# ChanganVR/RelationalGraphLearning

Hardware: AMD Instinct MI355X
Metric: agent-graph forward evals/sec (N=20, 2-layer GCN, depth-2 tree) (higher is better)
Workload: dtype f32 (24-bit operands throughout; 13 312 of the 14 224 products of the children kernel's 32 x 32, 32 x 100 and 100 x 100 head matrices, its embedding / graph weight products (w_r's second layer, Wa, W1, W_last) and the state predictor's weight products as six bf16 MFMA terms over three round-to-neare

## Files before the change

include/rgl_hip.h:

```cpp
#ifndef RGL_HIP_H
#define RGL_HIP_H

#include <stddef.h>

#ifdef __cplusplus
extern "C" {
#endif

#define RGL_ABI_VERSION 8

#define RGL_MAX_MLP_LAYERS 6
#define RGL_MAX_GCN_LAYERS 8
#define RGL_MAX_NODES 128
#define RGL_MAX_XDIM 64
#define RGL_MAX_WIDTH 256
#define RGL_MAX_ACTIONS 256

#define RGL_OK 0
#define RGL_ERR_BAD_SHAPE (-1)
#define RGL_ERR_BAD_MODE (-2)
#define RGL_ERR_NULL (-3)
#define RGL_ERR_WORKSPACE (-4)
#define RGL_CONTRACT_F32 0
#define RGL_CONTRACT_F16 1
// ... 123 lines not shown
    int planning_width;
    int do_action_clip;
    int sparse_search;
    int contraction_dtype;
    double time_step;
    double gamma_bar;
    const double* actions;
    const int* action_groups;
    const double* root_robot_f64;
    const double* root_humans_f64;
    const float* children_image;
    const float* predictor_image;
    double action_speed_bound;
} MprlPlanner;

size_t mprl_children_image_bytes(const MprlPlanner* planner);
int mprl_pack_children_image_f32(const MprlPlanner* planner, float* image, size_t image_bytes, rgl_stream_t stream);
size_t mprl_predictor_image_bytes(const MprlPlanner* planner);
int mprl_pack_predictor_image_f32(const MprlPlanner* planner, float* image, size_t image_bytes, rgl_stream_t stream);

int mprl_expand_f32(const MprlPlanner* planner, const float* robot, const float* humans, int P, int H,
                    int parents_are_joint_states,
                    float* humans_next, float* child_robot, float* reward, float* child_value,
                    float* value1, void* workspace, size_t workspace_bytes, rgl_stream_t stream);

size_t mprl_value_children_workspace_bytes(const MprlPlanner* planner, int P, int H);
int mprl_value_children_f32(const MprlPlanner* planner, const float* child_robot, const float* humans_next,
                            int P, int H, float* child_value, void* workspace, size_t workspace_bytes,
                            rgl_stream_t stream);

// ... 86 lines not shown
```

relationalgraphlearning_amd/_native.py:

```python
import ctypes as C
import os

_HERE = os.path.dirname(os.path.abspath(__file__))
LIB_PATH = os.environ.get("RGL_HIP_LIBRARY") or os.path.join(_HERE, "lib", "librgl_hip.so")

MAX_MLP_LAYERS = 6
MAX_GCN_LAYERS = 8
MAX_NODES = 128
MAX_XDIM = 64
MAX_WIDTH = 256
MAX_ACTIONS = 256
ABI_VERSION = 8
MSE_WORKSPACE_BYTES = 2048

SIMILARITY = {"embedded_gaussian": 0, "gaussian": 1, "cosine": 2, "cosine_softmax": 3, "concatenation": 4,
              "squared": 5, "equal_attention": 6, "diagonal": 7}
KINEMATICS = {"holonomic": 0, "unicycle": 1}
CONTRACTION_DTYPES = {"f32": 0, "f16": 1, "bf16x6": 3}

ERRORS = {-1: "RGL_ERR_BAD_SHAPE", -2: "RGL_ERR_BAD_MODE", -3: "RGL_ERR_NULL", -4: "RGL_ERR_WORKSPACE",
          -5: "RGL_ERR_LDS"}

c_float_p = C.POINTER(C.c_float)
c_int_p = C.POINTER(C.c_int)
# ... 9 lines not shown
    _fields_ = [("src", C.c_void_p), ("dst", C.c_void_p), ("rows", C.c_int), ("cols", C.c_int)]


class RglGatherJob(C.Structure):
    _fields_ = [("src", C.c_void_p), ("dst", C.c_void_p), ("row_floats", C.c_int), ("src_rows", C.c_int)]


class RglRowsPlan(C.Structure):
    _fields_ = [("kind", C.c_int), ("coop", C.c_int), ("waves_per_wg", C.c_int), ("n_waves", C.c_int), ("n_tiles", C.c_int),
                ("n_wgs", C.c_int), ("direct", C.c_int), ("reserved", C.c_int), ("lds_bytes", C.c_size_t)]


class RglGraphTilesPlan(C.Structure):
    _fields_ = [("covered", C.c_int), ("node_tiles", C.c_int), ("feature_tiles", C.c_int), ("layers", C.c_int), ("family", C.c_int),
                ("norm", C.c_int), ("grid", C.c_int), ("resident", C.c_int), ("lds_bytes", C.c_size_t)]


class RglGraph(C.Structure):
    _fields_ = [("w_r", RglMlp), ("w_h", RglMlp), ("x_dim", C.c_int), ("num_layer", C.c_int),
                ("similarity", C.c_int), ("layerwise_graph", C.c_int), ("skip_connection", C.c_int),
                ("reserved", C.c_int), ("w_a", C.c_void_p), ("w_a_mlp", RglMlp),
                ("Ws", C.c_void_p * MAX_GCN_LAYERS)]


class GcnPlanner(C.Structure):
    _fields_ = [("graph", RglGraph), ("value_head", RglMlp), ("kinematics", C.c_int), ("num_actions", C.c_int),
                ("time_step", C.c_double), ("gamma", C.c_double), ("actions", C.c_void_p),
                ("root_robot_f64", C.c_void_p), ("root_humans_f64", C.c_void_p), ("contraction_dtype", C.c_int), ("reserved", C.c_int)]


# ... 39 lines not shown


SIGNATURES = {
    "rgl_graph_forward_workspace_bytes": (C.c_size_t, [C.POINTER(RglGraph), C.POINTER(RglMlp), C.POINTER(RglMlp), C.c_int,
                                                       C.c_int, C.c_int]),
    "rgl_graph_forward_f32": (C.c_int, [C.POINTER(RglGraph), C.POINTER(RglMlp), C.POINTER(RglMlp), C.c_void_p,
                                        C.c_void_p, C.c_int, C.c_int, C.c_int, C.c_void_p, C.c_void_p, C.c_void_p,
                                        C.c_void_p, C.c_void_p, C.c_size_t, C.c_void_p]),
    "rgl_graph_param_count": (C.c_int, [C.POINTER(RglGraph), C.POINTER(RglMlp), C.POINTER(RglMlp)]),
    "rgl_graph_backward_workspace_bytes": (C.c_size_t, [C.POINTER(RglGraph), C.POINTER(RglMlp), C.POINTER(RglMlp), C.c_int]),
    "rgl_graph_backward_f32": (C.c_int, [C.POINTER(RglGraph), C.POINTER(RglMlp), C.POINTER(RglMlp), C.c_void_p, C.c_void_p,
                                         C.c_int, C.c_int, C.c_int, C.c_void_p, C.c_void_p, C.c_void_p, C.c_void_p,
                                         C.c_void_p, C.c_size_t, C.c_void_p]),
    "rgl_plan_mlp_rows": (C.c_int, [C.POINTER(RglMlp), C.c_int, C.c_int, C.POINTER(RglRowsPlan)]),
    "rgl_plan_graph_tiles": (C.c_int, [C.POINTER(RglGraph), C.c_int, C.c_int, C.c_int, C.c_int, C.POINTER(RglGraphTilesPlan)]),
    "rgl_transpose_f32": (C.c_int, [C.c_void_p, C.c_void_p, C.c_int, C.c_int, C.c_void_p]),
    "rgl_transpose_many_f32": (C.c_int, [C.c_void_p, C.c_int, C.c_void_p]),
    "rgl_gather_rows_f32": (C.c_int, [C.c_void_p, C.c_int, C.c_void_p, C.c_int, C.c_void_p]),
    "rgl_mse_step_f32": (C.c_int, [C.c_void_p, C.c_void_p, C.c_void_p, C.c_void_p, C.c_float, C.c_int, C.c_void_p, C.c_void_p,
                                   C.c_void_p, C.c_void_p]),
    "gcn_rotate_f32": (C.c_int, [C.c_void_p, C.c_void_p, C.c_int, C.c_int, C.c_void_p]),
    "gcn_prepare_f32": (C.c_int, [C.POINTER(GcnPlanner), C.c_void_p, C.c_void_p, C.c_int, C.c_int, C.c_void_p, C.c_void_p,
                                  C.c_void_p, C.c_void_p]),
    "gcn_predict_workspace_bytes": (C.c_size_t, [C.c_int, C.c_int, C.c_int]),
    "gcn_predict_f32": (C.c_int, [C.POINTER(GcnPlanner), C.c_void_p, C.c_void_p, C.c_int, C.c_int, C.c_void_p,
                                  C.c_size_t, C.c_void_p, C.c_void_p, C.c_void_p, C.c_void_p]),
    "mprl_expand_f32": (C.c_int, [C.POINTER(MprlPlanner), C.c_void_p, C.c_void_p, C.c_int, C.c_int, C.c_int,
                                  C.c_void_p, C.c_void_p, C.c_void_p, C.c_void_p, C.c_void_p, C.c_void_p, C.c_size_t,
                                  C.c_void_p]),
    "mprl_value_children_workspace_bytes": (C.c_size_t, [C.POINTER(MprlPlanner), C.c_int, C.c_int]),
# ... 17 lines not shown
    "mprl_tree_level_view": (C.c_int, [C.POINTER(MprlPlanner), C.c_int, C.c_int, C.c_int, C.POINTER(MprlLevelView)]),
    "crowd_step_f64": (C.c_int, [C.POINTER(CrowdSimConfig), C.c_void_p, C.c_void_p, C.c_void_p, C.c_void_p, C.c_void_p,
                                 C.c_void_p, C.c_void_p, C.c_void_p, C.c_int, C.c_int, C.c_int, C.c_void_p, C.c_void_p,
                                 C.c_void_p, C.c_void_p]),
    "crowd_observe_f32": (C.c_int, [C.c_void_p, C.c_void_p, C.c_int, C.c_int, C.c_void_p, C.c_void_p, C.c_void_p]),
    "crowd_orca_humans_f64": (C.c_int, [C.POINTER(CrowdOrcaParams), C.c_void_p, C.c_void_p, C.c_void_p, C.c_void_p,
                                        C.c_void_p, C.c_int, C.c_int, C.c_int, C.c_void_p, C.c_void_p]),
    "crowd_orca_robot_f64": (C.c_int, [C.POINTER(CrowdOrcaParams), C.c_void_p, C.c_void_p, C.c_void_p, C.c_int, C.c_int,
                                       C.c_void_p, C.c_void_p]),
    "crowd_generate_scenes_f64": (C.c_int, [C.POINTER(CrowdSceneConfig), C.c_void_p, C.c_int, C.c_int, C.c_void_p, C.c_void_p,
                                            C.c_void_p, C.c_void_p, C.c_void_p, C.c_void_p, C.c_void_p]),
    "rgl_abi_version": (C.c_int, []),
    "rgl_build_target": (C.c_char_p, []),
}

_lib = None


class NativeLibraryError(RuntimeError):
    pass


def lib():
    global _lib
    if _lib is None:
        if not os.path.exists(LIB_PATH):
            raise NativeLibraryError(
                "librgl_hip.so is not built (%s). Run `python -c 'import __graft_entry__ as g; g.build()'` or "
                "`make -C relationalgraphlearning_amd/csrc`. There is no CPU fallback." % LIB_PATH)
        handle = C.CDLL(LIB_PATH)
        for name, (res, args) in SIGNATURES.items():
            try:
                fn = getattr(handle, name)
            except AttributeError as e:
                raise NativeLibraryError("librgl_hip.so lacks symbol %s" % name) from e
            fn.restype = res
            fn.argtypes = args
        if handle.rgl_abi_version() != ABI_VERSION:
            raise NativeLibraryError("librgl_hip.so ABI %d != expected %d" % (handle.rgl_abi_version(), ABI_VERSION))
        _lib = handle
    return _lib


def poison_workspaces():
    return os.environ.get("RGL_DEBUG_POISON_WORKSPACES", "0") == "1"


def check(rc, what):
    if rc == 0:
# ... 5 lines not shown
```

relationalgraphlearning_amd/csrc/rgl_common.h:

```cpp
#pragma once
#include <hip/hip_runtime.h>

#include <cstdlib>

#include "rgl_hip.h"

#define RGL_HIP_TRY(expr)                          \
    do {                                           \
        hipError_t e__ = (expr);                   \
        if (e__ != hipSuccess) return (int)e__;    \
    } while (0)

#define RGL_LAUNCH_CHECK()                         \
    do {                                           \
        hipError_t e__ = hipGetLastError();        \
        if (e__ != hipSuccess) return (int)e__;    \
    } while (0)

namespace rgl {

constexpr int kLdsBytesPerCu = 160 * 1024;

inline int validate_mlp(const RglMlp& m, int want_in, int want_out) {
    if (m.n_layers < 1 || m.n_layers > RGL_MAX_MLP_LAYERS) return RGL_ERR_BAD_SHAPE;
// ... 57 lines not shown
                         hipStream_t stream, int mode = 0);
size_t fused_children_workspace_bytes(int P, int A, int H);
const float* fused_workspace_image(const void* workspace, size_t workspace_bytes);
int launch_value_children(const MprlPlanner* pl, const float* child_robot, const float* humans_next, int P, int H,
                          float* child_value, void* workspace, size_t workspace_bytes, hipStream_t stream,
                          int image_ready = 0, const void* tail = nullptr, size_t tail_bytes = 0,
                          int* tail_done = nullptr, const void* prologue = nullptr, size_t prologue_bytes = 0);
size_t value_children_workspace_bytes(const MprlPlanner* pl, int P, int H);
int launch_predict_humans(const MprlPlanner* pl, const float* robot, const float* humans, int crowds_per, int P, int H,
                          float* humans_next, void* workspace, size_t workspace_bytes, hipStream_t stream,
                          const void* children = nullptr, size_t children_bytes = 0, int* children_done = nullptr,
                          const float* sp_image = nullptr);
int level_prologue_args(const MprlPlanner* pl, const float* robot, const float* humans, int crowds_per, int P, int H,
                        float* humans_next, const float* sp_image, const void* children, size_t children_bytes, void* out,
                        size_t out_bytes);
bool fused_prologue_fits(const MprlPlanner* pl, int P, int H, size_t workspace_bytes, int scene_floats);
size_t scene_image_bytes(const MprlPlanner* pl);
int pack_scene_image(const MprlPlanner* pl, float* image, hipStream_t stream);
size_t scene_image_bytes_for(const RglGraph& g, const RglMlp* motion_head);
int pack_scene_image_for(const RglGraph& g, const RglMlp* motion_head, float* image, hipStream_t stream);

int launch_scene_children(const MprlPlanner* pl, const float* child_robot, const float* humans_next, int P, int H,
                          float* child_value, void* workspace, size_t workspace_bytes, hipStream_t stream);
size_t scene_children_workspace_bytes(int P, int A, int H);

int launch_backward_mfma(const RglGraph* graph, const RglMlp* value_head, const RglMlp* motion_head, const float* robot,
                         const float* humans, int n_scenes, int H, int detach_graph, const float* d_value,
                         const float* d_humans_next, const float* d_H, float* grad_out, void* workspace, size_t workspace_bytes,
                         hipStream_t stream, int only_choice);

// ... 48 lines not shown
```

relationalgraphlearning_amd/csrc/rgl_fused.hip:

```cpp
#include "rgl_mlp_chain.h"
#include "rgl_scene_body.h"
#include "rgl_tail.h"

#include <mutex>
#include <unordered_map>
#include <vector>

namespace {

__host__ __device__ constexpr bool fused_packed_rows(int HR, bool SOFT) { return SOFT && HR <= 20; }
__host__ __device__ constexpr int fused_scratch_floats(int HR, int NT, bool SOFT) {
    const int NP = 16 * NT, HRL = HR < NP ? HR : NP;
    const int main_fl = fused_packed_rows(HR, SOFT) ? HRL * 32 + 16 * (HRL + 2) * 2 : 2 * 16 * (NP + 1) + 16 * XLD;
    const int crowd_fl = NP * XLD + 2 * NP;
    const int fl = main_fl > crowd_fl ? main_fl : crowd_fl;
    return ((fl > kTailLdsInts ? fl : kTailLdsInts) + 3) & ~3;
}

struct FusedArgs {
    const float *wr1, *br1, *wr2, *br2, *wa, *w1;
    const float *wh1, *bh1, *wh2, *bh2;
    const float* w_last;
    const float *hw1, *hb1, *hw2, *hb2, *hw3, *hb3, *hw4, *hb4;
    const float* child_robot;
// ... 364 lines not shown
        load_fence();
        __builtin_amdgcn_wave_barrier();
    };
    static_assert(LO::scratch % 4 == 0 && LO::f_last % 4 == 0, "b128 granules");
    constexpr int kChunk = 256;
    constexpr int kChunksA = (LO::f_last + kChunk - 1) / kChunk, kChunksAll = (LO::scratch + kChunk - 1) / kChunk;
    int* image_arrivals = reinterpret_cast<int*>(lds + LO::scratch + kFusedWaves * fused_scratch_floats(HR, NT, SOFT));
    auto image_chunk = [&](int c) {
        const int fl = c * kChunk + lane * 4;
        if (fl < LO::scratch)
            __builtin_amdgcn_global_load_lds((const __attribute__((address_space(1))) void*)(a.image + fl),
                                             (__attribute__((address_space(3))) void*)(lds + c * kChunk), 16, 0, 0);
    };
    if constexpr (PRO) {
        static_assert(kPrologueSceneBase<LO> == kChunksA * kChunk, "the scene region starts behind the first part's chunks");
        for (int c = wave; c < kChunksA; c += kFusedWaves) image_chunk(c);
        scene_body<2, 0, kFusedWaves, false, true, true>(pa.scene, lds + kPrologueSceneBase<LO>, p_first, 1, kFusedWaves, p_first + k_b);
        const ChildrenArgs& ca = pa.children;
        const long long pair0 = (long long)p_first * ca.A, pair_end = (long long)(p_first + k_b) * ca.A;
        if (ca.A >= 64 && ca.H <= 64 && !ca.robot64) {
            const float v_max = table_speed_bound(ca);
            for (long long base = pair0 + 64 * wave; base < pair_end; base += 64 * kFusedWaves) children_wave(ca, base, pair_end, v_max);
        } else {
            for (long long idx = pair0 + tid; idx < pair_end; idx += nthreads) children_thread(ca, idx);
        }
        __syncthreads();
        wh2_loads();
    }
    if (wave < n_items) item_loads(item_at(0));
    if (tid == 0) *image_arrivals = 0;
    bool image_complete = false;
    if (a.image_sync) {
        copy_image<LO::scratch, nthreads>(lds, a.image, tid);
        __syncthreads();
        image_complete = true;
    } else {
    if (!PRO) for (int c = wave; c < kChunksA; c += kFusedWaves) image_chunk(c);
    __builtin_amdgcn_s_waitcnt(0x0F70);
    __syncthreads();
    for (int c = kChunksA + wave; c < kChunksAll; c += kFusedWaves) image_chunk(c);
    }
// ... 804 lines not shown
    fp.a.image_sync = image_sync;
    static const int phase_delay = env_int("RGL_FUSED_PHASE_DELAY", 0), prio = env_int("RGL_FUSED_PRIO", 2);
    fp.a.phase_delay = phase_delay;
    fp.a.prio = prio;
    if (ta) {
        fp.a.tail = *ta;
        fp.a.tail.chain = chain;
    }
    const int rc = launch_fused(fp, g->skip_connection != 0, stream);
    if (rc == RGL_OK && ta && tail_done) *tail_done = chain ? 2 : 1;
    return rc;
}

constexpr int kPrologueMinParentsPerCu = 4;

bool fused_prologue_fits(const MprlPlanner* pl, int P, int H, size_t workspace_bytes, int scene_floats) {
    if (pl->contraction_dtype != RGL_CONTRACT_BF16X6 || head_variant(pl->value_head) < 0) return false;
    if (P < kPrologueMinParentsPerCu * fused_cu_count() - (fused_cu_count() - 1)) return false;
    if (workspace_bytes < value_children_workspace_bytes(pl, P, H)) return false;
    return prologue_form(plan_fused(pl->value_graph, pl->value_head, P, pl->num_actions, H, 1, kModeBx), scene_floats);
}

}

static bool head_image_args(const RglGraph& g, const RglMlp& head, FusedArgs& a) {
    if (!fast_path_enabled() || g.x_dim != XD || g.num_layer < 2 || g.num_layer > RGL_MAX_GCN_LAYERS) return false;
    if (!mlp_is(g.w_r, 9, HID, XD, true) || !mlp_is(g.w_h, 5, HID, XD, true) || head_variant(head) != 0) return false;
    a = FusedArgs{};
    a.wr1 = g.w_r.weight[0]; a.br1 = g.w_r.bias[0]; a.wr2 = g.w_r.weight[1]; a.br2 = g.w_r.bias[1];
    a.wa = bilinear_wa(g); a.w1 = g.Ws[0];
    a.w_last = g.Ws[g.num_layer - 1];
    a.hw1 = head.weight[0]; a.hb1 = head.bias[0]; a.hw2 = head.weight[1]; a.hb2 = head.bias[1];
    a.hw3 = head.weight[2]; a.hb3 = head.bias[2]; a.hw4 = head.weight[3]; a.hb4 = head.bias[3];
    a.wh1 = g.w_h.weight[0]; a.bh1 = g.w_h.bias[0]; a.wh2 = g.w_h.weight[1]; a.bh2 = g.w_h.bias[1];
    return true;
}

// ... 24 lines not shown
```

relationalgraphlearning_amd/csrc/rgl_scene.hip:

```cpp
#include "rgl_scene_body.h"

namespace {

struct RowMlpArgs {
    const float *w1, *b1, *w2, *b2;
    const float* rows;
    float* out;
    int M, n_tiles;
};

template <int IN>
__device__ __forceinline__ void row_mlp2_tiles(const RowMlpArgs& a, const float* lds_set, int first, int stride, int lane) {
    constexpr int F1 = 0, F2 = F1 + 4 * 1 * 4 * 64, B1 = F2 + 2 * 4 * 4 * 64, B2 = B1 + HID;
    const int n = lane & 15, q = lane >> 4;
    for (int tile = first; tile < a.n_tiles; tile += stride) {
        const int row = 16 * tile + n;
        const int rc = row < a.M ? row : a.M - 1;
        const float* src = a.rows + (size_t)rc * IN;
        f32x4 in[1];
#pragma unroll
        for (int r = 0; r < 4; ++r) {
            const int feat = tile_feature<IN>(0, q, r);
            in[0][r] = feat < IN ? src[feat] : 0.f;
        }
        f32x4 h[4];
        layer_mfma<IN, HID, true>(lds_set + F1, in, h, lane, lds_set + B1);
        relu_tiles<HID>(h);
        f32x4 o[2];
        layer_mfma<HID, XD, true>(lds_set + F2, h, o, lane, lds_set + B2);
        relu_tiles<XD>(o);
        if (row < a.M) {
            float* dst = a.out + (size_t)row * XD;
            *reinterpret_cast<f32x4*>(dst + 4 * q) = o[0];
            *reinterpret_cast<f32x4*>(dst + 16 + 4 * q) = o[1];
        }
    }
}

constexpr int kRowMlpSetFloats = 4 * 1 * 4 * 64 + 2 * 4 * 4 * 64 + HID + XD;

template <int INA, int INB>
__global__ __launch_bounds__(kThreads, 2) void row_mlp2_pair_kernel(const RowMlpArgs ra, const RowMlpArgs rb, int grid_a, int grid_mlp,
                                                                    const ChildrenArgs ca) {
    extern __shared__ __attribute__((aligned(16))) float lds[];
    if ((int)blockIdx.x >= grid_mlp) {
        const long long total = (long long)ca.P * ca.A, stride = (long long)(gridDim.x - grid_mlp) * kThreads;
        const long long first_pair = (long long)(blockIdx.x - grid_mlp) * kThreads + threadIdx.x;
        if (ca.A >= 64 && ca.H <= 64 && !ca.robot64) {
            const float v_max = table_speed_bound(ca);
            for (long long base = first_pair & ~63LL; base < total; base += stride) children_wave(ca, base, total, v_max);
        } else {
            for (long long idx = first_pair; idx < total; idx += stride) children_thread(ca, idx);
        }
        return;
// ... 20 lines not shown
    if constexpr (CH) {
        if ((int)blockIdx.x >= grid_scene) {
            const long long total = (long long)ca.P * ca.A, stride = (long long)(gridDim.x - grid_scene) * kSceneThreads;
            const long long first = (long long)(blockIdx.x - grid_scene) * kSceneThreads + threadIdx.x;
            if (ca.A >= 64 && ca.H <= 64 && !ca.robot64) {
                const float v_max = table_speed_bound(ca);
                for (long long base = first & ~63LL; base < total; base += stride) children_wave(ca, base, total, v_max);
            } else {
                for (long long idx = first; idx < total; idx += stride) children_thread(ca, idx);
            }
            return;
        }
    }
    extern __shared__ __attribute__((aligned(16))) float lds[];
    scene_body<NT, SK, WAVES, SPLIT, EMB, BX>(a, lds, blockIdx.x, grid_scene, grid_scene * kSlots, a.P);
}

struct SceneImageLayout { int off_wa, off_ws, off_wm1, off_bm1, off_wm2, off_bm2, total, ws_stride; };
inline SceneImageLayout scene_image_layout(int L, bool bx = false) {
    SceneImageLayout o;
    int off = 0;
    auto take = [&](int nfl) { int r = off; off += (nfl + 3) & ~3; return r; };
    o.ws_stride = bx ? B6Floats<XD, XD>::v : XD * WLD;
    o.off_wa = take(bx ? B6Floats<XD, XD>::v : XD * WLD);
    o.off_ws = take(L * o.ws_stride);
    o.off_wm1 = take(bx ? B6Floats<XD, HID>::v : XD * W1LD);
    o.off_bm1 = take(HID);
    o.off_wm2 = take(bx ? B6Floats<HID, 16>::v : HID * M2LD);
    o.off_bm2 = take(16);
    o.total = off;
    return o;
}

struct SceneImageArgs {
    const float* wa;
    const float* Ws[4];
    const float *wm1, *bm1, *wm2, *bm2;
    int L;
    SceneImageLayout lo;
};

__global__ __launch_bounds__(256) void scene_pack_b6_kernel(const SceneImageArgs a, float* img) {
    const int e = blockIdx.x * 256 + threadIdx.x;
    const SceneImageLayout& lo = a.lo;
    if (e >= lo.total) return;
    float v = 0.f;
// ... 119 lines not shown
}

}

namespace {

static bool scene_kernel_covers(const RglGraph& g, int N) {
    const bool path_m = mlp_is(g.w_r, 9, HID, XD, true) && mlp_is(g.w_h, 5, HID, XD, true);
    const bool path_g = mlp_is(g.w_r, 6, HID, XD, true) && mlp_is(g.w_h, 7, HID, XD, true);
    return fast_path_enabled() && scene_similarity_mode(g) >= 0 && g.x_dim == XD && g.num_layer >= 1 && g.num_layer <= 4 &&
           (path_m || path_g) && N <= 128 && (N <= 64 || scene_similarity_mode(g) != SIM_CONCAT);
}

static int fill_scene_args(SceneArgs& sa, const RglGraph& g, const RglMlp* mh, const float* robot, const float* humans, int crowds_per,
                           int P, int H, float* humans_next, float* rows_out, float* x0_rows, float* xh_rows, bool embed_inside,
                           const float* sp_image, int slots);

static int run_scene_kernels(const RglGraph& g, const RglMlp* mh, const float* robot, const float* humans, int crowds_per, int P,
                             int H, float* humans_next, float* rows_out, float* x0_rows, float* xh_rows,
                             const ChildrenArgs* ca, hipStream_t stream, const ChildrenArgs* embed_children = nullptr,
                             const float* sp_image = nullptr) {
    const int N = H + 1, n_crowds = P / crowds_per;
    const int NT0 = N > 64 ? 8 : (N + 15) / 16;
    static const bool emb_off = [] { const char* e = getenv("RGL_SCENE_EMBED_INSIDE"); return e && e[0] == '0'; }();
    const bool embed_inside = !emb_off && !embed_children && g.w_r.dims[0] == 9 && scene_similarity_mode(g) == SIM_SOFTMAX &&
                              (NT0 == 1 || NT0 == 2 || NT0 == 4) && P <= 512 &&
                              (NT0 == 1 || P < scene_split_below(NT0));
    if (!embed_inside) {
        int rc = launch_row_mlp2_pair(g.w_r, robot, x0_rows, P, g.w_h, humans, xh_rows, n_crowds * H, stream, embed_children);
        if (rc) return rc;
    }
    SceneArgs sa;
    const size_t lds_bytes = fill_scene_args(sa, g, mh, robot, humans, crowds_per, P, H, humans_next, rows_out, x0_rows, xh_rows,
                                             embed_inside, sp_image, 0) * sizeof(float);
    switch (NT0) {
        case 1: return launch_scene<1, 8>(sa, lds_bytes, ca, stream);
        case 2: return launch_scene<2, 8>(sa, lds_bytes, ca, stream);
        case 3: return launch_scene<3, 4>(sa, lds_bytes, ca, stream);
        case 4: return launch_scene<4, 4>(sa, lds_bytes, ca, stream);
        default: return launch_scene_wide(sa, lds_bytes, ca, stream);
    }
}

static int fill_scene_args(SceneArgs& sa, const RglGraph& g, const RglMlp* mh, const float* robot, const float* humans, int crowds_per,
                           int P, int H, float* humans_next, float* rows_out, float* x0_rows, float* xh_rows, bool embed_inside,
                           const float* sp_image, int slots) {
    const int N = H + 1;
    const int NT = N > 64 ? 8 : (N + 15) / 16;
    sa.robot_rows = embed_inside ? robot : nullptr;
    sa.human_rows = embed_inside ? humans : nullptr;
    sa.er_w1 = g.w_r.weight[0]; sa.er_b1 = g.w_r.bias[0]; sa.er_w2 = g.w_r.weight[1]; sa.er_b2 = g.w_r.bias[1];
    sa.eh_w1 = g.w_h.weight[0]; sa.eh_b1 = g.w_h.bias[0]; sa.eh_w2 = g.w_h.weight[1]; sa.eh_b2 = g.w_h.bias[1];
    sa.off_er = sa.off_eh = 0;
    const bool split_ok = sp_image && scene_similarity_mode(g) == SIM_SOFTMAX && NT == 2 && g.num_layer <= 4;
    sa.bx = split_ok ? 1 : 0;
    sa.image = sp_image;
    sa.xh_rows = xh_rows; sa.x0_rows = x0_rows; sa.crowds_per = crowds_per;
    sa.wa = bilinear_wa(g);
    sa.sim = scene_similarity_mode(g);
    sa.layerwise = g.layerwise_graph;
    for (int l = 0; l < RGL_MAX_GCN_LAYERS; ++l) sa.Ws[l] = l < g.num_layer ? g.Ws[l] : nullptr;
// ... 13 lines not shown
        sa.image_floats = lo.total;
        off = lo.total;
    }
    sa.wc1 = sa.bc1 = sa.wc2 = sa.bc2 = nullptr;
    sa.off_wc1 = sa.off_bc1 = sa.off_wc2 = 0;
    if (sa.sim == SIM_CONCAT) {
        sa.wc1 = g.w_a_mlp.weight[0]; sa.bc1 = g.w_a_mlp.bias[0]; sa.wc2 = g.w_a_mlp.weight[1]; sa.bc2 = g.w_a_mlp.bias[1];
        sa.off_wc1 = take(2 * XD * W1LD); sa.off_bc1 = take(HID); sa.off_wc2 = take(HID);
    }
    if (embed_inside) {
        sa.off_er = take(kRowMlpSetFloats);
        sa.off_eh = take(kRowMlpSetFloats);
    }
    sa.wave_stride = 16 * NT * XLD;
    static const bool wide_slots = [] { const char* e = getenv("RGL_SCENE_WIDE_SLOTS"); return e && e[0] == '1'; }();
    if (slots <= 0) slots = (embed_inside && (NT == 2 || NT == 4) && !wide_slots) ? 8 / NT : (NT <= 2 ? 8 : (NT <= 4 ? 4 : 1));
    sa.off_wave = take(slots * sa.wave_stride);
    return off;
}

}

namespace rgl {

size_t scene_image_bytes_for(const RglGraph& g, const RglMlp* mh) {
    if (!scene_kernel_covers(g, 20) || scene_similarity_mode(g) != SIM_SOFTMAX) return 0;
    if (mh && !mlp_is(*mh, XD, HID, 5, false)) return 0;
    return (((size_t)scene_image_layout(g.num_layer, true).total * sizeof(float)) + 255) & ~(size_t)255;
}

size_t scene_image_bytes(const MprlPlanner* pl) {
    if (!pl || pl->linear_state_predictor) return 0;
// ... 12 lines not shown
    ia.wa = bilinear_wa(g);
    for (int l = 0; l < 4; ++l) ia.Ws[l] = l < g.num_layer ? g.Ws[l] : nullptr;
    ia.wm1 = mh ? mh->weight[0] : nullptr; ia.bm1 = mh ? mh->bias[0] : nullptr;
    ia.wm2 = mh ? mh->weight[1] : nullptr; ia.bm2 = mh ? mh->bias[1] : nullptr;
    ia.L = g.num_layer;
    ia.lo = scene_image_layout(g.num_layer, true);
    hipLaunchKernelGGL(scene_pack_b6_kernel, dim3((ia.lo.total + 255) / 256), dim3(256), 0, stream, ia, image);
    RGL_LAUNCH_CHECK();
    return RGL_OK;
}

int level_prologue_args(const MprlPlanner* pl, const float* robot, const float* humans, int crowds_per, int P, int H,
                        float* humans_next, const float* sp_image, const void* children, size_t children_bytes, void* out,
                        size_t out_bytes) {
    if (!out || out_bytes != sizeof(LevelPrologue) || !children || children_bytes != sizeof(ChildrenArgs)) return 1;
    if (pl->linear_state_predictor || pl->contraction_dtype != RGL_CONTRACT_BF16X6 || !sp_image) return 1;
    const RglGraph& g = pl->predictor_graph;
    const int N = H + 1;
    if (!scene_kernel_covers(g, N) || !mlp_is(pl->motion_head, XD, HID, 5, false) || g.w_r.dims[0] != 9) return 1;
    if (scene_similarity_mode(g) != SIM_SOFTMAX || (N + 15) / 16 != 2 || crowds_per < 1 || P % crowds_per != 0) return 1;
    LevelPrologue* lp = (LevelPrologue*)out;
    lp->scene_floats = fill_scene_args(lp->scene, g, &pl->motion_head, robot, humans, crowds_per, P, H, humans_next, nullptr, nullptr,
                                       nullptr, true, sp_image, 8);
    if (!lp->scene.bx) return 1;
    lp->children = *(const ChildrenArgs*)children;
    return 0;
}

int launch_predict_humans(const MprlPlanner* pl, const float* robot, const float* humans, int crowds_per, int P, int H,
                          float* humans_next, void* workspace, size_t workspace_bytes, hipStream_t stream,
                          const void* children, size_t children_bytes, int* children_done, const float* sp_image) {
    const ChildrenArgs* ca = (children && children_bytes == sizeof(ChildrenArgs)) ? (const ChildrenArgs*)children : nullptr;
    if (children_done) *children_done = 0;
    const RglGraph& g = pl->predictor_graph;
    const RglMlp& mh = pl->motion_head;
    const int N = H + 1;
    const bool ok = scene_kernel_covers(g, N) && mlp_is(mh, XD, HID, 5, false) && workspace &&
                    workspace_bytes >= (size_t)P * N * XD * sizeof(float) && P % crowds_per == 0;
    if (!ok) {
        if (P % crowds_per == 0) {
// ... 79 lines not shown
```

relationalgraphlearning_amd/csrc/rgl_scene_body.h:

```cpp
#pragma once
#include "rgl_children.h"
#include "rgl_mlp_chain.h"

namespace {

struct SceneArgs {
    const float* robot_rows;
    const float* human_rows;
    const float *er_w1, *er_b1, *er_w2, *er_b2;
    const float *eh_w1, *eh_b1, *eh_w2, *eh_b2;
    int off_er, off_eh;
    int bx;
    int ws_stride;
    int image_floats;
    const float* image;
    const float* xh_rows;
    const float* x0_rows;
    int crowds_per;
    const float* wa;
    const float* Ws[RGL_MAX_GCN_LAYERS];
    int L, skip;
    int sim;
    const float *wm1, *bm1, *wm2, *bm2;
    float* humans_next;
    float* rows_out;
    int layerwise;
    const float *wc1, *bc1, *wc2, *bc2;
    int off_wc1, off_bc1, off_wc2;
    int P, H, N;
    int off_wa, off_ws, off_wm1, off_bm1, off_wm2, off_bm2, off_wave, wave_stride;
};

struct LevelPrologue {
    SceneArgs scene;
    ChildrenArgs children;
    int scene_floats;
};

constexpr int M2LD = 20;

template <int NT, int SK, int WAVES, bool SPLIT, bool EMB = false, bool BX = false>
__device__ __forceinline__ void scene_body(const SceneArgs& a, float* lds, int first, int slot_step, int pass_step, int end) {
    static_assert(!BX || SK == 0, "six-term bf16 products: softmax similarity");
    static_assert(!SPLIT || (SK != 3 && NT > 1 && WAVES % NT == 0), "split scenes: whole scenes per workgroup, no pair-MLP similarity");
    constexpr int kSceneThreads = WAVES * 64;
    constexpr int NCT = SPLIT ? 1 : NT;
    const int sim = SK == 0 ? (int)SIM_SOFTMAX : a.sim;
    const int tid = threadIdx.x, lane = tid & 63, wave = tid >> 6;
    const int n = lane & 15, q = lane >> 4;
    const int N = a.N, H = a.H;
    const float* wa = lds + a.off_wa;
    const float* ws = lds + a.off_ws;
    const float* wm1 = lds + a.off_wm1;
    const float* bm1 = lds + a.off_bm1;
    const float* wm2 = lds + a.off_wm2;
    const float* bm2 = lds + a.off_bm2;
    const int slot = __builtin_amdgcn_readfirstlane(SPLIT ? wave / NT : wave);
    const int ctb = SPLIT ? __builtin_amdgcn_readfirstlane(wave % NT) : 0;
// ... 76 lines not shown
    }
    if constexpr (EMB) {
        float* w = lds;
        constexpr int F1 = 0, F2 = F1 + 4 * 1 * 4 * 64, B1 = F2 + 2 * 4 * 4 * 64, B2 = B1 + HID;
        if constexpr (BX) emb_loads();
        frag_store(er1, w + a.off_er + F1, tid);
        frag_store(er2, w + a.off_er + F2, tid);
        bias_store<HID>(ebias[0], w + a.off_er + B1, tid);
        bias_store<XD>(ebias[1], w + a.off_er + B2, tid);
        frag_store(eh1, w + a.off_eh + F1, tid);
        frag_store(eh2, w + a.off_eh + F2, tid);
        bias_store<HID>(ebias[2], w + a.off_eh + B1, tid);
        bias_store<XD>(ebias[3], w + a.off_eh + B2, tid);
    }
    __syncthreads();
    for (int it = first + (SPLIT ? 0 : slot_step * slot); it < end; it += pass_step) {
        const int sc_raw = SPLIT ? it + slot_step * slot : it;
        const bool active = sc_raw < end;
        const int sc = active ? sc_raw : end - 1;
        if constexpr (EMB) {
            constexpr int F1 = 0, F2 = F1 + 4 * 1 * 4 * 64, B1 = F2 + 2 * 4 * 4 * 64, B2 = B1 + HID;
            const float* er = lds + a.off_er;
            const float* eh = lds + a.off_eh;
#pragma unroll
            for (int ct = 0; ct < NCT; ++ct) {
                const int node = 16 * (ct + ctb) + n;
                const bool human = node >= 1 && node < N;
                const float* hsrc = a.human_rows + ((size_t)(sc / a.crowds_per) * H + (human ? node - 1 : 0)) * 5;
                f32x4 in[1];
#pragma unroll
                for (int r = 0; r < 4; ++r) {
                    const int feat = tile_feature<5>(0, q, r);
                    in[0][r] = (human && feat < 5) ? hsrc[feat] : 0.f;
                }
                f32x4 hh[4], oh[2];
// ... 8 lines not shown
                        const int feat = tile_feature<9>(0, q, r);
                        in[0][r] = (n == 0 && feat < 9) ? rsrc[feat] : 0.f;
                    }
                    f32x4 orr[2];
                    layer_mfma<9, HID, true>(er + F1, in, hh, lane, er + B1);
                    relu_tiles<HID>(hh);
                    layer_mfma<HID, XD, true>(er + F2, hh, orr, lane, er + B2);
                    relu_tiles<XD>(orr);
                    if (n == 0) { oh[0] = orr[0]; oh[1] = orr[1]; }
                }
#pragma unroll
                for (int ot = 0; ot < 2; ++ot)
                    *reinterpret_cast<f32x4*>(&Hs[node * XLD + 16 * ot + 4 * q]) = node < N ? oh[ot] : zero4();
            }
            __builtin_amdgcn_wave_barrier();
        } else {
        const float* xr = a.x0_rows + (size_t)sc * XD;
        const float* xh = a.xh_rows + (size_t)(sc / a.crowds_per) * H * XD;
        for (int idx = lane; idx < 16 * NCT * (XD / 4); idx += 64) {
            const int row = (idx >> 3) + 16 * ctb, c4 = (idx & 7) * 4;
            f32x4 val = zero4();
            if (row == 0) val = *reinterpret_cast<const f32x4*>(xr + c4);
            else if (row < N) val = *reinterpret_cast<const f32x4*>(xh + (size_t)(row - 1) * XD + c4);
            *reinterpret_cast<f32x4*>(&Hs[row * XLD + c4]) = val;
        }
        }
        if (SPLIT) __syncthreads();
        constexpr bool PERM = SK != 3;
        auto jnode = [&](int jt, int r) { return 16 * jt + ((PERM && jt == NT - 1) ? 4 * r + q : 4 * q + r); };
        const int last_steps = PERM ? (N - 16 * (NT - 1) + 3) >> 2 : 4;
        f32x4 pr[NT][NT];
        auto adjacency = [&]() {
            if constexpr (SK == 3) {
                const float* wc1 = lds + a.off_wc1;
                const float* bc1 = lds + a.off_bc1;
                const float* wc2 = lds + a.off_wc2;
                const float bc2 = a.bc2[0];
                f32x4 pt[NT][4], qt[NT][4];
#pragma unroll
                for (int ct = 0; ct < NT; ++ct) {
#pragma unroll
// ... 244 lines not shown
                    }
                    const int node = 16 * (ct + ctb) + n;
                    if (active && node >= 1 && node < N) {
                        float* dst = a.humans_next + ((size_t)sc * H + (node - 1)) * 5;
#pragma unroll
                        for (int r = 0; r < 4; ++r) {
                            const int oidx = 4 * q + r;
                            if (oidx < 5) dst[oidx] = om[r] + bm2[oidx];
                        }
                    }
                }
            }
            if (SPLIT) __syncthreads(); else __builtin_amdgcn_wave_barrier();
        }
        if (SPLIT) __syncthreads();
    }
}

}
```

Before: 2.118 billion.

## Compute prologue human/robot embeddings cooperatively per workgroup chunk in LDS

In the fused level prologue, the state-predictor scene body no longer embeds each scene's human and robot rows per wave. It now processes parents in chunks, and all waves of the workgroup compute the crowd's human embeddings once per crowd and the robot embeddings once per parent into a shared LDS row buffer. Each scene then copies its rows from that buffer. This removes embedding work that was repeated when several parents share a crowd, and it spreads the embedding MFMAs across waves. The cost is extra workgroup barriers per chunk and LDS space for the row buffer. It also adds a planning query, optional phase-timing instrumentation and a compile-time fallback to the per-wave path.

```diff
diff --git a/include/rgl_hip.h b/include/rgl_hip.h
--- a/include/rgl_hip.h
+++ b/include/rgl_hip.h
@@ -161,6 +161,11 @@
     double action_speed_bound;
 } MprlPlanner;
 
+typedef struct RglPrologueEmbeddingPlan {
+    int prologue, parents_per_wg, workgroups, chunk_parents, chunk_crowds, human_tiles, robot_tiles, row_floats, chunks_per_wg, reserved;
+} RglPrologueEmbeddingPlan;
+int rgl_plan_prologue_embedding(const MprlPlanner* planner, int P, int H, int crowds_per, int unit, RglPrologueEmbeddingPlan* plan);
+
 size_t mprl_children_image_bytes(const MprlPlanner* planner);
 int mprl_pack_children_image_f32(const MprlPlanner* planner, float* image, size_t image_bytes, rgl_stream_t stream);
 size_t mprl_predictor_image_bytes(const MprlPlanner* planner);
diff --git a/relationalgraphlearning_amd/_native.py b/relationalgraphlearning_amd/_native.py
--- a/relationalgraphlearning_amd/_native.py
+++ b/relationalgraphlearning_amd/_native.py
@@ -47,6 +47,11 @@
 class RglGraphTilesPlan(C.Structure):
     _fields_ = [("covered", C.c_int), ("node_tiles", C.c_int), ("feature_tiles", C.c_int), ("layers", C.c_int), ("family", C.c_int),
                 ("norm", C.c_int), ("grid", C.c_int), ("resident", C.c_int), ("lds_bytes", C.c_size_t)]
+
+
+class RglPrologueEmbeddingPlan(C.Structure):
+    _fields_ = [(n, C.c_int) for n in ("prologue", "parents_per_wg", "workgroups", "chunk_parents", "chunk_crowds", "human_tiles",
+                                       "robot_tiles", "row_floats", "chunks_per_wg", "reserved")]
 
 
 class RglGraph(C.Structure):
@@ -116,6 +121,7 @@
                                          C.c_void_p, C.c_size_t, C.c_void_p]),
     "rgl_plan_mlp_rows": (C.c_int, [C.POINTER(RglMlp), C.c_int, C.c_int, C.POINTER(RglRowsPlan)]),
     "rgl_plan_graph_tiles": (C.c_int, [C.POINTER(RglGraph), C.c_int, C.c_int, C.c_int, C.c_int, C.POINTER(RglGraphTilesPlan)]),
+    "rgl_plan_prologue_embedding": (C.c_int, [C.POINTER(MprlPlanner), C.c_int, C.c_int, C.c_int, C.c_int, C.POINTER(RglPrologueEmbeddingPlan)]),
     "rgl_transpose_f32": (C.c_int, [C.c_void_p, C.c_void_p, C.c_int, C.c_int, C.c_void_p]),
     "rgl_transpose_many_f32": (C.c_int, [C.c_void_p, C.c_int, C.c_void_p]),
     "rgl_gather_rows_f32": (C.c_int, [C.c_void_p, C.c_int, C.c_void_p, C.c_int, C.c_void_p]),
@@ -163,6 +169,8 @@
     "rgl_build_target": (C.c_char_p, []),
 }
 
+ADDITIVE = {"rgl_plan_prologue_embedding"}
+
 _lib = None
 
 
@@ -182,6 +190,8 @@
             try:
                 fn = getattr(handle, name)
             except AttributeError as e:
+                if name in ADDITIVE:
+                    continue
                 raise NativeLibraryError("librgl_hip.so lacks symbol %s" % name) from e
             fn.restype = res
             fn.argtypes = args
diff --git a/relationalgraphlearning_amd/csrc/rgl_common.h b/relationalgraphlearning_amd/csrc/rgl_common.h
--- a/relationalgraphlearning_amd/csrc/rgl_common.h
+++ b/relationalgraphlearning_amd/csrc/rgl_common.h
@@ -95,6 +95,8 @@
 int level_prologue_args(const MprlPlanner* pl, const float* robot, const float* humans, int crowds_per, int P, int H,
                         float* humans_next, const float* sp_image, const void* children, size_t children_bytes, void* out,
                         size_t out_bytes);
+int level_prologue_layout(const MprlPlanner* pl, int crowds_per, int P, int H, int* scene_floats, int* chunk_crowds);
+int fused_prologue_region_floats();
 bool fused_prologue_fits(const MprlPlanner* pl, int P, int H, size_t workspace_bytes, int scene_floats);
 size_t scene_image_bytes(const MprlPlanner* pl);
 int pack_scene_image(const MprlPlanner* pl, float* image, hipStream_t stream);
diff --git a/relationalgraphlearning_amd/csrc/rgl_fused.hip b/relationalgraphlearning_amd/csrc/rgl_fused.hip
--- a/relationalgraphlearning_amd/csrc/rgl_fused.hip
+++ b/relationalgraphlearning_amd/csrc/rgl_fused.hip
@@ -402,8 +402,19 @@
     };
     if constexpr (PRO) {
         static_assert(kPrologueSceneBase<LO> == kChunksA * kChunk, "the scene region starts behind the first part's chunks");
+        static_assert(kPrologueSceneBase<LO> + prologue_scene_floats(2, 19) <= LO::scratch + kFusedWaves * fused_scratch_floats(HR, NT, SOFT) + 4,
+                      "a two-layer predictor's scene region with the row buffer of a full chunk (12 crowds of 19 humans, 16 robot rows) fits the kernel's LDS");
+        ProPhases pro_phases;
+        ProPhases* const pp = &pro_phases;
+        PRO_PHASE_START(pp);
         for (int c = wave; c < kChunksA; c += kFusedWaves) image_chunk(c);
-        scene_body<2, 0, kFusedWaves, false, true, true>(pa.scene, lds + kPrologueSceneBase<LO>, p_first, 1, kFusedWaves, p_first + k_b);
+#ifdef RGL_PROLOGUE_EMB_PER_WAVE
+        constexpr bool kWge = false;
+#else
+        constexpr bool kWge = true;
+#endif
+        scene_body<2, 0, kFusedWaves, false, true, true, kWge>(pa.scene, lds + kPrologueSceneBase<LO>, p_first, 1, kFusedWaves,
+                                                               p_first + k_b, pp);
         const ChildrenArgs& ca = pa.children;
         const long long pair0 = (long long)p_first * ca.A, pair_end = (long long)(p_first + k_b) * ca.A;
         if (ca.A >= 64 && ca.H <= 64 && !ca.robot64) {
@@ -412,7 +423,10 @@
         } else {
             for (long long idx = pair0 + tid; idx < pair_end; idx += nthreads) children_thread(ca, idx);
         }
+        PRO_PHASE_MARK(pp, 3);
         __syncthreads();
+        PRO_PHASE_MARK(pp, 4);
+        PRO_PHASE_FLUSH(pp);
         wh2_loads();
     }
     if (wave < n_items) item_loads(item_at(0));
@@ -1247,6 +1261,11 @@
 
 constexpr int kPrologueMinParentsPerCu = 4;
 
+int fused_prologue_region_floats() {
+    using LO = FusedLds<32, 100, 100, true>;
+    return LO::scratch + kFusedWaves * fused_scratch_floats(20, 2, true) + 4 - kPrologueSceneBase<LO>;
+}
+
 bool fused_prologue_fits(const MprlPlanner* pl, int P, int H, size_t workspace_bytes, int scene_floats) {
     if (pl->contraction_dtype != RGL_CONTRACT_BF16X6 || head_variant(pl->value_head) < 0) return false;
     if (P < kPrologueMinParentsPerCu * fused_cu_count() - (fused_cu_count() - 1)) return false;
@@ -1254,6 +1273,30 @@
     return prologue_form(plan_fused(pl->value_graph, pl->value_head, P, pl->num_actions, H, 1, kModeBx), scene_floats);
 }
 
+}
+
+extern "C" int rgl_plan_prologue_embedding(const MprlPlanner* planner, int P, int H, int crowds_per, int unit,
+                                           RglPrologueEmbeddingPlan* plan) {
+    if (!planner || !plan) return RGL_ERR_NULL;
+    if (P < 1 || H < 1 || crowds_per < 1 || unit < 1 || P % crowds_per) return RGL_ERR_BAD_SHAPE;
+    *plan = RglPrologueEmbeddingPlan{};
+    static const bool prologue_on = [] { const char* e = getenv("RGL_LEVEL_PROLOGUE"); return !(e && e[0] == '0'); }();
+    int scene_floats = 0, chunk_crowds = 0;
+    if (!prologue_on || rgl::level_prologue_layout(planner, crowds_per, P, H, &scene_floats, &chunk_crowds)) return RGL_OK;
+    if (!rgl::fused_prologue_fits(planner, P, H, ~(size_t)0, scene_floats)) return RGL_OK;
+    const FusedPlan fp = plan_fused(planner->value_graph, planner->value_head, P, planner->num_actions, H, unit, kModeBx);
+    const int k = fp.a.parents_per_wg;
+    const int c1 = prologue_chunk_end(0, k, crowds_per, chunk_crowds);
+    plan->prologue = 1;
+    plan->parents_per_wg = k;
+    plan->workgroups = fp.grid;
+    plan->chunk_parents = c1;
+    plan->chunk_crowds = chunk_crowds;
+    plan->human_tiles = (((c1 - 1) / crowds_per + 1) * H + 15) / 16;
+    plan->robot_tiles = 1;
+    plan->row_floats = prologue_row_floats(H, chunk_crowds);
+    for (int c0 = 0; c0 < k; c0 = prologue_chunk_end(c0, k, crowds_per, chunk_crowds)) ++plan->chunks_per_wg;
+    return RGL_OK;
 }
 
 static bool head_image_args(const RglGraph& g, const RglMlp& head, FusedArgs& a) {
diff --git a/relationalgraphlearning_amd/csrc/rgl_scene.hip b/relationalgraphlearning_amd/csrc/rgl_scene.hip
--- a/relationalgraphlearning_amd/csrc/rgl_scene.hip
+++ b/relationalgraphlearning_amd/csrc/rgl_scene.hip
@@ -11,24 +11,12 @@
 
 template <int IN>
 __device__ __forceinline__ void row_mlp2_tiles(const RowMlpArgs& a, const float* lds_set, int first, int stride, int lane) {
-    constexpr int F1 = 0, F2 = F1 + 4 * 1 * 4 * 64, B1 = F2 + 2 * 4 * 4 * 64, B2 = B1 + HID;
     const int n = lane & 15, q = lane >> 4;
     for (int tile = first; tile < a.n_tiles; tile += stride) {
         const int row = 16 * tile + n;
         const int rc = row < a.M ? row : a.M - 1;
-        const float* src = a.rows + (size_t)rc * IN;
-        f32x4 in[1];
-#pragma unroll
-        for (int r = 0; r < 4; ++r) {
-            const int feat = tile_feature<IN>(0, q, r);
-            in[0][r] = feat < IN ? src[feat] : 0.f;
-        }
-        f32x4 h[4];
-        layer_mfma<IN, HID, true>(lds_set + F1, in, h, lane, lds_set + B1);
-        relu_tiles<HID>(h);
         f32x4 o[2];
-        layer_mfma<HID, XD, true>(lds_set + F2, h, o, lane, lds_set + B2);
-        relu_tiles<XD>(o);
+        row_mlp2_tile<IN>(lds_set, a.rows + (size_t)rc * IN, lane, o);
         if (row < a.M) {
             float* dst = a.out + (size_t)row * XD;
             *reinterpret_cast<f32x4*>(dst + 4 * q) = o[0];
@@ -36,8 +24,6 @@
         }
     }
 }
-
-constexpr int kRowMlpSetFloats = 4 * 1 * 4 * 64 + 2 * 4 * 4 * 64 + HID + XD;
 
 template <int INA, int INB>
 __global__ __launch_bounds__(kThreads, 2) void row_mlp2_pair_kernel(const RowMlpArgs ra, const RowMlpArgs rb, int grid_a, int grid_mlp,
@@ -88,22 +74,6 @@
     }
     extern __shared__ __attribute__((aligned(16))) float lds[];
     scene_body<NT, SK, WAVES, SPLIT, EMB, BX>(a, lds, blockIdx.x, grid_scene, grid_scene * kSlots, a.P);
-}
-
-struct SceneImageLayout { int off_wa, off_ws, off_wm1, off_bm1, off_wm2, off_bm2, total, ws_stride; };
-inline SceneImageLayout scene_image_layout(int L, bool bx = false) {
-    SceneImageLayout o;
-    int off = 0;
-    auto take = [&](int nfl) { int r = off; off += (nfl + 3) & ~3; return r; };
-    o.ws_stride = bx ? B6Floats<XD, XD>::v : XD * WLD;
-    o.off_wa = take(bx ? B6Floats<XD, XD>::v : XD * WLD);
-    o.off_ws = take(L * o.ws_stride);
-    o.off_wm1 = take(bx ? B6Floats<XD, HID>::v : XD * W1LD);
-    o.off_bm1 = take(HID);
-    o.off_wm2 = take(bx ? B6Floats<HID, 16>::v : HID * M2LD);
-    o.off_bm2 = take(16);
-    o.total = off;
-    return o;
 }
 
 struct SceneImageArgs {
@@ -253,7 +223,7 @@
 
 static int fill_scene_args(SceneArgs& sa, const RglGraph& g, const RglMlp* mh, const float* robot, const float* humans, int crowds_per,
                            int P, int H, float* humans_next, float* rows_out, float* x0_rows, float* xh_rows, bool embed_inside,
-                           const float* sp_image, int slots);
+                           const float* sp_image, int slots, int region_floats = 0);
 
 static int run_scene_kernels(const RglGraph& g, const RglMlp* mh, const float* robot, const float* humans, int crowds_per, int P,
                              int H, float* humans_next, float* rows_out, float* x0_rows, float* xh_rows,
@@ -283,7 +253,7 @@
 
 static int fill_scene_args(SceneArgs& sa, const RglGraph& g, const RglMlp* mh, const float* robot, const float* humans, int crowds_per,
                            int P, int H, float* humans_next, float* rows_out, float* x0_rows, float* xh_rows, bool embed_inside,
-                           const float* sp_image, int slots) {
+                           const float* sp_image, int slots, int region_floats) {
     const int N = H + 1;
     const int NT = N > 64 ? 8 : (N + 15) / 16;
     sa.robot_rows = embed_inside ? robot : nullptr;
@@ -327,8 +297,15 @@
     }
     sa.wave_stride = 16 * NT * XLD;
     static const bool wide_slots = [] { const char* e = getenv("RGL_SCENE_WIDE_SLOTS"); return e && e[0] == '1'; }();
+    const bool prologue = slots > 0;
     if (slots <= 0) slots = (embed_inside && (NT == 2 || NT == 4) && !wide_slots) ? 8 / NT : (NT <= 2 ? 8 : (NT <= 4 ? 4 : 1));
     sa.off_wave = take(slots * sa.wave_stride);
+    sa.off_rows = sa.chunk_crowds = 0;
+    if (prologue) {
+        const int room = (region_floats - off - kPrologueChunk * XD) / (H * XD);
+        sa.chunk_crowds = room < kPrologueChunkCrowds ? room : kPrologueChunkCrowds;
+        sa.off_rows = take(prologue_row_floats(H, sa.chunk_crowds > 0 ? sa.chunk_crowds : 1));
+    }
     return off;
 }
 
@@ -371,16 +348,28 @@
                         float* humans_next, const float* sp_image, const void* children, size_t children_bytes, void* out,
                         size_t out_bytes) {
     if (!out || out_bytes != sizeof(LevelPrologue) || !children || children_bytes != sizeof(ChildrenArgs)) return 1;
-    if (pl->linear_state_predictor || pl->contraction_dtype != RGL_CONTRACT_BF16X6 || !sp_image) return 1;
+    if (!sp_image || level_prologue_layout(pl, crowds_per, P, H, nullptr, nullptr)) return 1;
+    LevelPrologue* lp = (LevelPrologue*)out;
+    lp->scene_floats = fill_scene_args(lp->scene, pl->predictor_graph, &pl->motion_head, robot, humans, crowds_per, P, H, humans_next,
+                                       nullptr, nullptr, nullptr, true, sp_image, 8, fused_prologue_region_floats());
+    if (!lp->scene.bx) return 1;
+    lp->children = *(const ChildrenArgs*)children;
+    return 0;
+}
+
+int level_prologue_layout(const MprlPlanner* pl, int crowds_per, int P, int H, int* scene_floats, int* chunk_crowds) {
+    if (pl->linear_state_predictor || pl->contraction_dtype != RGL_CONTRACT_BF16X6) return 1;
     const RglGraph& g = pl->predictor_graph;
     const int N = H + 1;
     if (!scene_kernel_covers(g, N) || !mlp_is(pl->motion_head, XD, HID, 5, false) || g.w_r.dims[0] != 9) return 1;
     if (scene_similarity_mode(g) != SIM_SOFTMAX || (N + 15) / 16 != 2 || crowds_per < 1 || P % crowds_per != 0) return 1;
-    LevelPrologue* lp = (LevelPrologue*)out;
-    lp->scene_floats = fill_scene_args(lp->scene, g, &pl->motion_head, robot, humans, crowds_per, P, H, humans_next, nullptr, nullptr,
-                                       nullptr, true, sp_image, 8);
-    if (!lp->scene.bx) return 1;
-    lp->children = *(const ChildrenArgs*)children;
+    SceneArgs sa;
+    static const float image_stand_in = 0.f;
+    const int fl = fill_scene_args(sa, g, &pl->motion_head, nullptr, nullptr, crowds_per, P, H, nullptr, nullptr, nullptr, nullptr, true,
+                                   &image_stand_in, 8, fused_prologue_region_floats());
+    if (!sa.bx || sa.chunk_crowds < 1) return 1;
+    if (scene_floats) *scene_floats = fl;
+    if (chunk_crowds) *chunk_crowds = sa.chunk_crowds;
     return 0;
 }
 
diff --git a/relationalgraphlearning_amd/csrc/rgl_scene_body.h b/relationalgraphlearning_amd/csrc/rgl_scene_body.h
--- a/relationalgraphlearning_amd/csrc/rgl_scene_body.h
+++ b/relationalgraphlearning_amd/csrc/rgl_scene_body.h
@@ -13,6 +13,7 @@
     int bx;
     int ws_stride;
     int image_floats;
+    int off_rows;
     const float* image;
     const float* xh_rows;
     const float* x0_rows;
@@ -21,6 +22,7 @@
     const float* Ws[RGL_MAX_GCN_LAYERS];
     int L, skip;
     int sim;
+    int chunk_crowds;
     const float *wm1, *bm1, *wm2, *bm2;
     float* humans_next;
     float* rows_out;
@@ -39,9 +41,82 @@
 
 constexpr int M2LD = 20;
 
-template <int NT, int SK, int WAVES, bool SPLIT, bool EMB = false, bool BX = false>
-__device__ __forceinline__ void scene_body(const SceneArgs& a, float* lds, int first, int slot_step, int pass_step, int end) {
+constexpr int kPrologueChunk = 16, kPrologueChunkCrowds = 12;
+__host__ __device__ inline int prologue_chunk_end(int c0, int end, int crowds_per, int max_crowds) {
+    int c1 = c0 + kPrologueChunk;
+    const int by_crowds = (c0 / crowds_per + max_crowds) * crowds_per;
+    if (by_crowds < c1) c1 = by_crowds;
+    return c1 < end ? c1 : end;
+}
+constexpr int prologue_row_floats(int H, int max_crowds) { return (max_crowds * H + kPrologueChunk) * XD; }
+
+struct SceneImageLayout { int off_wa, off_ws, off_wm1, off_bm1, off_wm2, off_bm2, total, ws_stride; };
+constexpr SceneImageLayout scene_image_layout(int L, bool bx = false) {
+    SceneImageLayout o{};
+    int off = 0;
+    auto take = [&](int nfl) { int r = off; off += (nfl + 3) & ~3; return r; };
+    o.ws_stride = bx ? B6Floats<XD, XD>::v : XD * WLD;
+    o.off_wa = take(bx ? B6Floats<XD, XD>::v : XD * WLD);
+    o.off_ws = take(L * o.ws_stride);
+    o.off_wm1 = take(bx ? B6Floats<XD, HID>::v : XD * W1LD);
+    o.off_bm1 = take(HID);
+    o.off_wm2 = take(bx ? B6Floats<HID, 16>::v : HID * M2LD);
+    o.off_bm2 = take(16);
+    o.total = off;
+    return o;
+}
+
+constexpr int kRowMlpSetFloats = 4 * 1 * 4 * 64 + 2 * 4 * 4 * 64 + HID + XD;
+constexpr int prologue_scene_floats(int L, int H) {
+    return scene_image_layout(L, true).total + 2 * kRowMlpSetFloats + 8 * 32 * XLD + prologue_row_floats(H, kPrologueChunkCrowds);
+}
+
+#ifdef RGL_PHASE_TIMING
+struct ProPhases { unsigned long long acc[5] = {0, 0, 0, 0, 0}, t0 = 0; };
+#define PRO_PHASE_START(pp) do { if (pp) (pp)->t0 = __builtin_amdgcn_s_memtime(); } while (0)
+#define PRO_PHASE_MARK(pp, idx)                                            \
+    do {                                                                   \
+        if (pp) {                                                          \
+            const unsigned long long now__ = __builtin_amdgcn_s_memtime(); \
+            (pp)->acc[idx] += now__ - (pp)->t0;                            \
+            (pp)->t0 = now__;                                              \
+        }                                                                  \
+    } while (0)
+#define PRO_PHASE_FLUSH(pp)                                                \
+    do {                                                                   \
+        if ((threadIdx.x & 63) == 0)                                       \
+            for (int i__ = 0; i__ < 5; ++i__) atomicAdd(&g_phase_cycles[10 + i__], (pp)->acc[i__]); \
+    } while (0)
+#else
+struct ProPhases {};
+#define PRO_PHASE_START(pp) do { } while (0)
+#define PRO_PHASE_MARK(pp, idx) do { } while (0)
+#define PRO_PHASE_FLUSH(pp) do { (void)(pp); } while (0)
+#endif
+
+template <int IN>
+__device__ __forceinline__ void row_mlp2_tile(const float* lds_set, const float* src, int lane, f32x4 (&o)[2]) {
+    constexpr int F1 = 0, F2 = F1 + 4 * 1 * 4 * 64, B1 = F2 + 2 * 4 * 4 * 64, B2 = B1 + HID;
+    const int q = lane >> 4;
+    f32x4 in[1];
+#pragma unroll
+    for (int r = 0; r < 4; ++r) {
+        const int feat = tile_feature<IN>(0, q, r);
+        in[0][r] = feat < IN ? src[feat] : 0.f;
+    }
+    f32x4 h[4];
+    layer_mfma<IN, HID, true>(lds_set + F1, in, h, lane, lds_set + B1);
+    relu_tiles<HID>(h);
+    layer_mfma<HID, XD, true>(lds_set + F2, h, o, lane, lds_set + B2);
+    relu_tiles<XD>(o);
+}
+
+
+template <int NT, int SK, int WAVES, bool SPLIT, bool EMB = false, bool BX = false, bool WGE = false>
+__device__ __forceinline__ void scene_body(const SceneArgs& a, float* lds, int first, int slot_step, int pass_step, int end,
+                                           ProPhases* pp = nullptr) {
     static_assert(!BX || SK == 0, "six-term bf16 products: softmax similarity");
+    static_assert(!WGE || (EMB && !SPLIT), "workgroup-cooperative embeddings: the embedding sets in LDS, one scene per wave");
     static_assert(!SPLIT || (SK != 3 && NT > 1 && WAVES % NT == 0), "split scenes: whole scenes per workgroup, no pair-MLP similarity");
     constexpr int kSceneThreads = WAVES * 64;
     constexpr int NCT = SPLIT ? 1 : NT;
@@ -148,11 +223,47 @@
         bias_store<XD>(ebias[3], w + a.off_eh + B2, tid);
     }
     __syncthreads();
-    for (int it = first + (SPLIT ? 0 : slot_step * slot); it < end; it += pass_step) {
+    PRO_PHASE_MARK(pp, 0);
+    if (WGE && first >= end) return;
+    int c0 = first;
+    do {
+    const int c1 = WGE ? prologue_chunk_end(c0, end, a.crowds_per, a.chunk_crowds) : end;
+    const int cr0 = WGE ? c0 / a.crowds_per : 0;
+    const int robot_rows0 = WGE ? a.off_rows + a.chunk_crowds * H * XD : 0;
+    if constexpr (WGE) {
+        if (c0 != first) {
+            __syncthreads();
+            PRO_PHASE_MARK(pp, 4);
+        }
+        const int hrows = ((c1 - 1) / a.crowds_per - cr0 + 1) * H, htiles = (hrows + 15) >> 4;
+        for (int t = wave; t <= htiles; t += WAVES) {
+            f32x4 o[2];
+            int dst;
+            bool valid;
+            if (t < htiles) {
+                const int row = 16 * t + n;
+                valid = row < hrows;
+                row_mlp2_tile<5>(lds + a.off_eh, a.human_rows + ((size_t)cr0 * H + (valid ? row : hrows - 1)) * 5, lane, o);
+                dst = a.off_rows + row * XD;
+            } else {
+                valid = n < c1 - c0;
+                row_mlp2_tile<9>(lds + a.off_er, a.robot_rows + (size_t)(valid ? c0 + n : c1 - 1) * 9, lane, o);
+                dst = robot_rows0 + n * XD;
+            }
+            if (valid) {
+                *reinterpret_cast<f32x4*>(&lds[dst + 4 * q]) = o[0];
+                *reinterpret_cast<f32x4*>(&lds[dst + 16 + 4 * q]) = o[1];
+            }
+        }
+        PRO_PHASE_MARK(pp, 1);
+        __syncthreads();
+        PRO_PHASE_MARK(pp, 4);
+    }
+    for (int it = c0 + (SPLIT ? 0 : slot_step * slot); it < c1; it += pass_step) {
         const int sc_raw = SPLIT ? it + slot_step * slot : it;
-        const bool active = sc_raw < end;
-        const int sc = active ? sc_raw : end - 1;
-        if constexpr (EMB) {
+        const bool active = sc_raw < c1;
+        const int sc = active ? sc_raw : c1 - 1;
+        if constexpr (EMB && !WGE) {
             constexpr int F1 = 0, F2 = F1 + 4 * 1 * 4 * 64, B1 = F2 + 2 * 4 * 4 * 64, B2 = B1 + HID;
             const float* er = lds + a.off_er;
             const float* eh = lds + a.off_eh;
@@ -191,6 +302,17 @@
                     *reinterpret_cast<f32x4*>(&Hs[node * XLD + 16 * ot + 4 * q]) = node < N ? oh[ot] : zero4();
             }
             __builtin_amdgcn_wave_barrier();
+        } else if constexpr (WGE) {
+        const int xr = robot_rows0 + (sc - c0) * XD;
+        const int xh = a.off_rows + (sc / a.crowds_per - cr0) * H * XD;
+        for (int idx = lane; idx < 16 * NCT * (XD / 4); idx += 64) {
+            const int row = (idx >> 3) + 16 * ctb, c4 = (idx & 7) * 4;
+            f32x4 val = zero4();
+            if (row == 0) val = *reinterpret_cast<const f32x4*>(&lds[xr + c4]);
+            else if (row < N) val = *reinterpret_cast<const f32x4*>(&lds[xh + (row - 1) * XD + c4]);
+            *reinterpret_cast<f32x4*>(&Hs[row * XLD + c4]) = val;
+        }
+        __builtin_amdgcn_wave_barrier();
         } else {
         const float* xr = a.x0_rows + (size_t)sc * XD;
         const float* xh = a.xh_rows + (size_t)(sc / a.crowds_per) * H * XD;
@@ -202,6 +324,7 @@
             *reinterpret_cast<f32x4*>(&Hs[row * XLD + c4]) = val;
         }
         }
+        PRO_PHASE_MARK(pp, 1);
         if (SPLIT) __syncthreads();
         constexpr bool PERM = SK != 3;
         auto jnode = [&](int jt, int r) { return 16 * jt + ((PERM && jt == NT - 1) ? 4 * r + q : 4 * q + r); };
@@ -476,7 +599,10 @@
             if (SPLIT) __syncthreads(); else __builtin_amdgcn_wave_barrier();
         }
         if (SPLIT) __syncthreads();
+        PRO_PHASE_MARK(pp, 2);
     }
+    c0 = c1;
+    } while (WGE && c0 < end);
 }
 
 }
```

New measurement: 2.168 billion (median of 6 runs). 2.3% higher.
